# PieSil/CUDA-spectral-ray-tracer

Measured on AMD Instinct MI355X. Metric: Mray/s, higher is better.
Workload: dtype f32; 1 GPU; random-spheres tri scene (4802 tris, 9603 BVH nodes), 1920x1080, 1024 spp, depth 16; scene_id=100, tiles=8x8 px per wave, rank = tile % n_gpus, gather=none (1 GPU), launch_mode=one process, one GPU

## Files before the change

cuda-spectral-ray-tracer_amd/binding.py:

```python
import ctypes as C
import os

_HERE = os.path.dirname(os.path.abspath(__file__))
LIB_PATH = os.environ.get("SRT_LIB_PATH") or os.path.join(_HERE, "libsrt_hip.so")

N_CIE = 95
TILE_PLANES = 9
TILE_LANES = 64

SCENE_CORNELL, SCENE_PRISM, SCENE_TRIS, SCENE_RANDOM_SPHERES, SCENE_MESH100K = 0, 1, 2, 100, 101
BVH_REFERENCE, BVH_SAH = 0, 1
MAT_LAMBERTIAN, MAT_METALLIC, MAT_DIELECTRIC, MAT_EMISSIVE, MAT_NO_MAT = 0, 1, 2, 4, 6


class TriIn(C.Structure):
    _fields_ = [("v0", C.c_float * 3), ("v1", C.c_float * 3), ("v2", C.c_float * 3),
                ("mat_index", C.c_uint32), ("aa_plane", C.c_uint32)]


class Material(C.Structure):
    _fields_ = [("col", C.c_float * 3), ("reflection_fuzz", C.c_float), ("material_type", C.c_uint32),
                ("spectral_distribution", C.c_float * N_CIE), ("emission_power", C.c_float),
                ("sellmeier_B", C.c_float * 3), ("sellmeier_C", C.c_float * 3)]

# ... 118 lines not shown
    "srt_denoise_estimate_last_ms": (_i, [_vp, _fp]),
    "srt_denoise_features_mv": (_i, [_vp, C.POINTER(DenoiseVG), _fp, _fp, _fp, _fp, _u32, _u32]),
    "srt_denoise_mv_kat": (_i, [_vp, C.POINTER(DenoiseVG), _fp, _fp, C.POINTER(_u32), _fp, _u32, _u32, _fp, _fp]),
    "srt_accum_reset_streams": (_i, [_vp, _u32]),
    "srt_accum_streams": (_i, [_vp, C.POINTER(_u32)]),
    "srt_set_gather_planes": (_i, [_vp, _u32]),
    "srt_tile_buffer": (_i, [_vp, C.POINTER(_vp), C.POINTER(_sz), C.POINTER(_u32), C.POINTER(_u32)]),
    "srt_copy_tile_buffer": (_i, [_vp, _vp, _vp]),
    "srt_scatter_tiles": (_i, [_vp, _vp, _vp]),
    "srt_dev_fb": (_i, [_vp, C.POINTER(_vp), C.POINTER(_vp), C.POINTER(_vp), C.POINTER(_sz)]),
    "srt_read_fb": (_i, [_vp, _fp, _fp, _fp]),
    "srt_read_fb_rowmajor": (_i, [_vp, _fp, _fp, _fp, _u32, _u32]),
    "srt_read_fb_aux": (_i, [_vp, _i, _fp, _fp, _fp]),
    "srt_get_tile_costs": (_i, [_vp, C.POINTER(C.c_uint32), _sz]),
    "srt_order_children_by_profile": (_i, [_vp, _vp, C.c_uint32, C.c_uint32, C.c_uint32, C.c_uint32, C.c_uint32, C.POINTER(C.c_uint32)]),
    "srt_pixels_per_lane": (_i, [_vp, _u32, _u32, _u32, C.POINTER(C.c_double)]),
    "srt_tune_tree_for_throughput": (_i, [_vp, _vp, _u32, _u32, _u32, _u32, _i, C.POINTER(TreeTuning)]),
    "srt_get_stats": (_i, [_vp, C.POINTER(Stats)]),
    "srt_set_count_traversal": (_i, [_vp, _i]),
    "srt_get_wave_debug": (_i, [_vp, C.POINTER(C.c_uint32), _sz]),
    "srt_last_kernel_ms": (_i, [_vp, C.POINTER(_f)]),
    "srt_trace_rays": (_i, [_vp, _fp, _sz, _fp]),
    "srt_device_op_sweep": (_i, [_vp, _i, _fp, _fp, _sz, _fp]),
    "srt_order_tiles_kat": (_i, [_vp, C.POINTER(_u32), _u32, _u32, _u32, _u32, C.POINTER(_u32), _sz, C.POINTER(_u32), C.POINTER(_u32)]),
    "srt_read_tile_schedule": (_i, [_vp, _i, C.POINTER(_u32), _sz, C.POINTER(TileScheduleInfo)]),
    "srt_calibrate": (_i, [_vp, _i, _u32, _u32, C.POINTER(Calibration)]),
    "srt_ctx_device": (_i, [_vp]),
    "srt_ctx_cu_count": (_i, [_vp]),
    "srt_comm_init_all": (_i, [C.POINTER(_i), _i, C.POINTER(_vp)]),
    "srt_comm_unique_id": (_i, [C.POINTER(C.c_ubyte)]),
    "srt_comm_init_rank": (_i, [_vp, C.POINTER(C.c_ubyte), _u32, _u32, C.POINTER(_vp)]),
    "srt_comm_available": (_i, []),
    "srt_comm_set_gather_planes": (_i, [_vp, _u32]),
    "srt_comm_last_gather_ms": (_i, [_vp, C.POINTER(_f)]),
    "srt_comm_destroy": (None, [_vp]),
    "srt_comm_last_error": (C.c_char_p, [_vp]),
    "srt_comm_world": (_u32, [_vp]),
    "srt_comm_local_count": (_u32, [_vp]),
    "srt_comm_ctx": (_vp, [_vp, _u32]),
    "srt_comm_root_ctx": (_vp, [_vp]),
    "srt_comm_upload_scene": (_i, [_vp, _vp]),
    "srt_comm_set_camera": (_i, [_vp, C.POINTER(CameraData)]),
    "srt_comm_init_device_params": (_i, [_vp, _u32, _u32, _u32, _u32, _u32, _u32, _u32, _u32, _u64]),
    "srt_render_frame_multi": (_i, [_vp, _u32, _u32, _u32, _u32]),
    "srt_comm_accum_reset": (_i, [_vp]),
    "srt_render_frame_multi_accum": (_i, [_vp, _u32, _u32, _u32, _u32, _u32]),
# ... 56 lines not shown
```

cuda-spectral-ray-tracer_amd/csrc/srt_capi.cpp:

```cpp
#include <dlfcn.h>
#include <hip/hip_runtime.h>
#include <stdint.h>
#include <stdlib.h>
#include <string.h>

#include <algorithm>
#include <cmath>
#include <cstddef>
#include <string>
#include <vector>

#include "srt_host.h"
#include "srt_internal.h"

using namespace srt;

#ifndef SRT_FRINGE_STRIDE_L2
#define SRT_FRINGE_STRIDE_L2 96
#endif
static constexpr uint32_t kFringeStrideL2 = SRT_FRINGE_STRIDE_L2;
static constexpr uint32_t kScoreShadeL2 = 320u, kScoreFringeL2 = 800u;

struct DeviceBuffer {
    void *ptr = nullptr;
// ... 1679 lines not shown
    RenderParams p;
    fill_params(c, p);
    HIP_TRY_AS(c, "srt_trace_rays", launch_trace(p, d_in.as<float>(), n, d_out.as<float>(), nullptr));
    HIP_TRY_AS(c, "srt_trace_rays", hipDeviceSynchronize());
    HIP_TRY_AS(c, "srt_trace_rays", hipMemcpy(out, d_out.ptr, 4 * n * sizeof(float), hipMemcpyDeviceToHost));
    return SRT_OK;
}

int srt_device_op_sweep(srt_ctx *c, int which, const float *a, const float *b, size_t n, float *out) {
    if (!c || !a || !b || !out) return fail(c, SRT_ERR_INVALID, "srt_device_op_sweep: null argument");
    if (n == 0) return SRT_OK;
    HIP_TRY(c, hipSetDevice(c->device));
    DeviceBuffer buf;
    HIP_TRY_AS(c, "srt_device_op_sweep", buf.reserve(3 * n * sizeof(float)));
    float *d = buf.as<float>();
    HIP_TRY_AS(c, "srt_device_op_sweep", hipMemcpy(d, a, n * sizeof(float), hipMemcpyHostToDevice));
    HIP_TRY_AS(c, "srt_device_op_sweep", hipMemcpy(d + n, b, n * sizeof(float), hipMemcpyHostToDevice));
    HIP_TRY_AS(c, "srt_device_op_sweep", launch_op_sweep(which, d, d + n, n, d + 2 * n, nullptr));
    HIP_TRY_AS(c, "srt_device_op_sweep", hipDeviceSynchronize());
    HIP_TRY_AS(c, "srt_device_op_sweep", hipMemcpy(out, d + 2 * n, n * sizeof(float), hipMemcpyDeviceToHost));
    return SRT_OK;
}

int srt_order_tiles_kat(srt_ctx *c, const uint32_t *cost, uint32_t n, uint32_t n_waves, uint32_t split_load_pct, uint32_t order_max_pct,
                        uint32_t *rows_out, size_t rows_cap, uint32_t *sorted_out, uint32_t *info_out) {
    if (!c || !cost || !rows_out || !sorted_out || !info_out) return fail(c, SRT_ERR_INVALID, "srt_order_tiles_kat: null argument");
    if (n == 0 || n > (1u << 20)) return fail(c, SRT_ERR_INVALID, "srt_order_tiles_kat: n must be in 1 .. 2^20");
    if (rows_cap < (size_t)n * 64 + 64) return fail(c, SRT_ERR_INVALID, "srt_order_tiles_kat: rows_cap must be at least 64 * n + 64 (the largest queue and 64 guard words)");
    HIP_TRY(c, hipSetDevice(c->device));
    DeviceBuffer d_cost, d_rows, d_sorted, d_info;
    HIP_TRY_AS(c, "srt_order_tiles_kat", d_cost.reserve(TileSchedule::cost_bytes(n)));
    HIP_TRY_AS(c, "srt_order_tiles_kat", d_rows.reserve(rows_cap * sizeof(uint32_t)));
    HIP_TRY_AS(c, "srt_order_tiles_kat", d_sorted.reserve(n * sizeof(uint32_t)));
    HIP_TRY_AS(c, "srt_order_tiles_kat", d_info.reserve(4 * sizeof(uint32_t)));
    HIP_TRY_AS(c, "srt_order_tiles_kat", hipMemcpy(d_cost.ptr, cost, TileSchedule::cost_bytes(n), hipMemcpyHostToDevice));
    HIP_TRY_AS(c, "srt_order_tiles_kat", hipMemset(d_rows.ptr, 0xff, rows_cap * sizeof(uint32_t)));
    HIP_TRY_AS(c, "srt_order_tiles_kat", hipMemset(d_sorted.ptr, 0xff, n * sizeof(uint32_t)));
    HIP_TRY_AS(c, "srt_order_tiles_kat", hipMemset(d_info.ptr, 0xff, 4 * sizeof(uint32_t)));
    HIP_TRY_AS(c, "srt_order_tiles_kat", launch_order_tiles(d_cost.as<uint32_t>(), d_sorted.as<uint32_t>(), d_rows.as<uint32_t>(), n, n_waves, split_load_pct,
                                                            d_info.as<uint32_t>(), order_max_pct, nullptr));
    HIP_TRY_AS(c, "srt_order_tiles_kat", hipDeviceSynchronize());
    HIP_TRY_AS(c, "srt_order_tiles_kat", hipMemcpy(rows_out, d_rows.ptr, rows_cap * sizeof(uint32_t), hipMemcpyDeviceToHost));
    HIP_TRY_AS(c, "srt_order_tiles_kat", hipMemcpy(sorted_out, d_sorted.ptr, n * sizeof(uint32_t), hipMemcpyDeviceToHost));
    HIP_TRY_AS(c, "srt_order_tiles_kat", hipMemcpy(info_out, d_info.ptr, 4 * sizeof(uint32_t), hipMemcpyDeviceToHost));
    return SRT_OK;
}
// ... 56 lines not shown
```

cuda-spectral-ray-tracer_amd/csrc/srt_device.h:

```cpp
#pragma once
#include <hip/hip_runtime.h>
#include <stdint.h>

#include "srt_color_consts.h"
#include "srt_powf.h"

namespace srt {

constexpr int kCieSamples = 95;
constexpr int kWavelengths = 7;
constexpr float kLambdaMin = 360.0f;
constexpr float kLambdaMax = 830.0f;
constexpr float kEpsilon = 0.0001f;
constexpr float kFltMax = 3.402823466e+38f;

__device__ __noinline__ static float dev_powf(float x, float y) { return srt_powf(x, y); }

struct V3 { float x, y, z; };
__device__ __forceinline__ V3 mk(float x, float y, float z) { V3 r; r.x = x; r.y = y; r.z = z; return r; }
__device__ __forceinline__ V3 operator+(V3 a, V3 b) { return mk(a.x + b.x, a.y + b.y, a.z + b.z); }
__device__ __forceinline__ V3 operator-(V3 a, V3 b) { return mk(a.x - b.x, a.y - b.y, a.z - b.z); }
__device__ __forceinline__ V3 operator-(V3 a) { return mk(-a.x, -a.y, -a.z); }
__device__ __forceinline__ V3 operator*(float t, V3 v) { return mk(t * v.x, t * v.y, t * v.z); }
__device__ __forceinline__ float dot(V3 a, V3 b) { return a.x * b.x + a.y * b.y + a.z * b.z; }
__device__ __forceinline__ float length_squared(V3 v) { return v.x * v.x + v.y * v.y + v.z * v.z; }
__device__ __forceinline__ V3 unit_vector(V3 v) { float k = 1.0f / sqrtf(length_squared(v)); return k * v; }
__device__ __forceinline__ V3 reflect(V3 v, V3 n) { return v - (2.0f * dot(v, n)) * n; }
__device__ __forceinline__ V3 refract(V3 uv, V3 n, float etai_over_etat) {
    float cos_theta = fminf(dot(-uv, n), 1.0f);
    V3 r_out_perp = etai_over_etat * (uv + cos_theta * n);
    V3 r_out_parallel = (-sqrtf(fabsf(1.0f - length_squared(r_out_perp)))) * n;
    return r_out_perp + r_out_parallel;
}

__device__ __forceinline__ float inside_min2(float a1, float a2, uint32_t sign) {
    return __builtin_elementwise_minimum(__uint_as_float(__float_as_uint(a1) ^ sign), __uint_as_float(__float_as_uint(a2) ^ sign));
}
__device__ __forceinline__ bool inside_min3(float m12, float a3, uint32_t sign) {
    return __builtin_elementwise_minimum(m12, __uint_as_float(__float_as_uint(a3) ^ sign)) >= 0.f;
}

__device__ __forceinline__ bool near_zero(V3 v) {
    const float s = 1e-8f;
    return (fabsf(v.x) < s) && (fabsf(v.y) < s) && (fabsf(v.z) < s);
}

struct Rng { uint32_t d, v0, v1, v2, v3, v4; };
#ifndef SRT_XOR3
#define SRT_XOR3 1
#endif
#ifndef SRT_ASM_RNG
#define SRT_ASM_RNG 1
#endif

// ... 94 lines not shown
        : "s80", "s81", "vcc");
}
__device__ __forceinline__ V3 random_in_unit_sphere(Rng &s) {
#if SRT_ASM_RNG
    {
        float x, y, z, len2;
        rng_sphere_loop_asm(s, x, y, z, len2);
        return mk(x, y, z);
    }
#endif
    for (;;) {
        float x = rng_pm1(s);
        float y = rng_pm1(s);
        float z = rng_pm1(s);
        V3 p = mk(x, y, z);
        if (length_squared(p) < 1.0f) return p;
    }
}

__device__ __forceinline__ V3 random_unit_vector(Rng &s) {
#if SRT_ASM_RNG
    float x, y, z, len2;
    rng_sphere_loop_asm(s, x, y, z, len2);
    const float k = 1.0f / sqrtf(len2);
    return k * mk(x, y, z);
#else
    return unit_vector(random_in_unit_sphere(s));
#endif
}

__device__ __forceinline__ void interp_coords(float lambda, int &offset, float &weight) {
    lambda -= kLambdaMin;
    lambda *= ((float)kCieSamples - 1) / (kLambdaMax - kLambdaMin);
    offset = (int)lambda;
    if (offset < 0) offset = 0;
    if (offset > kCieSamples - 2) offset = kCieSamples - 2;
    weight = lambda - (float)offset;
}
__device__ __forceinline__ float interp_pair(float2 pr, float weight) { return (1.0f - weight) * pr.x + weight * pr.y; }

__device__ __forceinline__ float hero_draw(Rng &s) { return rng_range(s, kLambdaMin, kLambdaMax); }
__device__ __forceinline__ void hero_expand(float hero, float (&wl)[kWavelengths]) {
    const float step = (kLambdaMax - kLambdaMin) / (float)kWavelengths;
    wl[0] = hero;
    float lambda = hero;
#pragma unroll
    for (int i = 1; i < kWavelengths; i++) {
// ... 7 lines not shown
}

__device__ __forceinline__ float correct_channel(float value) {
    return value < 0.0f ? 0.0f
         : (value < 0.0031308f ? 12.92f * value
         : (value < 1.0f ? ((1.055f * dev_powf(value, 0.416666f)) - 0.055f) : 1.0f));
}
struct SrgbPixel { V3 lin, q; };
__device__ __forceinline__ SrgbPixel xyz_mean_to_srgb(V3 c) {
    const float r_lin = (SRT_XYZ2RGB_00 * c.x) + (SRT_XYZ2RGB_01 * c.y) + (SRT_XYZ2RGB_02 * c.z);
    const float g_lin = (SRT_XYZ2RGB_10 * c.x) + (SRT_XYZ2RGB_11 * c.y) + (SRT_XYZ2RGB_12 * c.z);
    const float b_lin = (SRT_XYZ2RGB_20 * c.x) + (SRT_XYZ2RGB_21 * c.y) + (SRT_XYZ2RGB_22 * c.z);
    const float r = correct_channel(r_lin), g = correct_channel(g_lin), b = correct_channel(b_lin);
    SrgbPixel o;
    o.lin = mk(r, g, b);
    o.q = mk((float)(int)(r * 255.99f), (float)(int)(g * 255.99f), (float)(int)(b * 255.99f));
    return o;
}

__device__ __forceinline__ float sellmeier_index(float b0, float b1, float b2, float c0, float c1, float c2, float lambda) {
    lambda *= 1e-3f;
    float l2 = lambda * lambda;
    float index = 1.0f + (b0 * l2) / (l2 - c0) + (b1 * l2) / (l2 - c1) + (b2 * l2) / (l2 - c2);
    return sqrtf(index);
}
__device__ __forceinline__ float reflectance(float cosine, float ref_idx) {
    float r0 = (1.0f - ref_idx) / (1.0f + ref_idx);
    r0 = r0 * r0;
    return r0 + (1.0f - r0) * srt_pow5f(1.0f - cosine);
}

constexpr uint32_t kTriWIsY = 1u, kTriHIsZ = 2u, kTriClockwise = 4u;

__device__ __forceinline__ bool tri_test(const float4 *__restrict__ tris, int tri, V3 o, V3 d, float tmin, float tmax,
                                         float &t_out) {
    const float4 a = tris[3 * tri + 0];
    const V3 n = mk(a.x, a.y, a.z);
    float denom = dot(n, d);
    if (fabsf(denom) < 1e-8f) return false;
    float t = (a.w - dot(n, o)) / denom;
    if (!(tmin <= t && t <= tmax)) return false;
    const float4 b = tris[3 * tri + 1];
    const float4 c = tris[3 * tri + 2];
    const uint32_t flags = __float_as_uint(c.z);
    const bool wy = flags & kTriWIsY, hz = flags & kTriHIsZ;
    float pw = (wy ? o.y : o.x) + t * (wy ? d.y : d.x);
    float ph = (hz ? o.z : o.y) + t * (hz ? d.z : d.y);
// ... 554 lines not shown
```

cuda-spectral-ray-tracer_amd/csrc/srt_internal.h:

```cpp
#pragma once
#include <hip/hip_runtime.h>
#include <stdint.h>
#include <stddef.h>

struct srt_ctx;
extern "C" int srt_internal_init_device_params(srt_ctx *c, uint32_t tx, uint32_t ty, uint32_t bx, uint32_t by, uint32_t chunk_w, uint32_t chunk_h,
                                               uint32_t spp, uint32_t bounce_limit, uint64_t seed, int wait);

extern "C" uint32_t srt_internal_gather_planes(const srt_ctx *c);

namespace srt {

constexpr int kTilePlanes = 9;
constexpr int kTileGroups = 3;
constexpr int kGroupPlanes = 3;
constexpr int kTileLanes = 64;
constexpr int kCounters = 32;

constexpr uint32_t kQueueTileBits = 22, kQueueTileMask = (1u << kQueueTileBits) - 1u;
constexpr uint32_t kQueuePartShift = kQueueTileBits, kQueuePartMask = 63u;
constexpr uint32_t kQueueLevelShift = 28, kQueueLevelMask = 7u;

struct RenderParams {
    const float4 *nodes;
// ... 174 lines not shown
};
hipError_t launch_denoise_level_dev(const DenoiseLevelDevParams &p, hipStream_t st);
hipError_t launch_denoise_dev_out(const float4 *payload, float *out_dev, uint32_t channels, uint32_t groups, size_t n, hipStream_t st);
constexpr uint32_t kMaxDevelopChannels = 16;
struct DevelopParams {
    const float *film, *response;
    float *out;
    float scale;
    uint32_t channels;
    uint32_t n_lanes, tx, ty, bx;
    uint32_t w, h;
};
uint32_t develop_padded_channels(uint32_t channels);
hipError_t launch_develop(const DevelopParams &p, hipStream_t st);
hipError_t launch_develop_srgb(const float *xyz, float *out_lin, float *out_q, uint32_t samples, size_t n, hipStream_t st);
hipError_t launch_order_tiles(const uint32_t *cost, uint32_t *sorted, uint32_t *rows, uint32_t n, uint32_t n_waves,
                              uint32_t split_load_pct, uint32_t *queue_info, uint32_t order_max_pct, hipStream_t st);
hipError_t launch_scatter(const ScatterParams &p, hipStream_t st);
hipError_t launch_unswizzle(const float *const src[3], float *const dst[3], uint32_t tx, uint32_t ty, uint32_t bx, uint32_t by,
                            uint32_t n_cols, uint32_t n_rows, uint32_t offx, uint32_t offy, uint32_t image_width,
                            uint32_t image_height, hipStream_t st);
hipError_t launch_trace(const RenderParams &p, const float *rays, size_t n, float *out, hipStream_t st);
hipError_t launch_op_sweep(int which, const float *a, const float *b, size_t n, float *out, hipStream_t st);
hipError_t launch_calib(int kind, uint32_t n_blocks, uint32_t threads, uint32_t iters, float *sink, unsigned long long *cycles, const float4 *table,
                        uint32_t n_records, hipStream_t st);
int calib_kinds();
bool render_narrow_refs(int n_records, const PlanKnobs &k);
bool render_paired_variant(bool tree_is_paired, bool narrow, bool all_cached);
size_t render_lds_bytes(int stack_depth, int waves_per_block, int n_cached, int n_records, const PlanKnobs &k);
void render_launch_shape(int stack_depth, int n_records, int n_inner, const PlanKnobs &k, int &waves_per_block, int &n_cached);
struct LaunchPlan { int waves_per_block, blocks_per_cu, waves_per_cu, waves_per_eu, n_cached; bool all_cached; };
void render_launch_plan(int stack_depth, int n_records, int n_inner, const PlanKnobs &k, LaunchPlan &lp);
struct RenderGrid { int waves_per_block; uint32_t n_blocks, waves; };
RenderGrid render_launch_grid(const LaunchPlan &lp, uint32_t n_cu, uint32_t waves_per_cu_override, uint32_t queue_rows_bound);

}
```

cuda-spectral-ray-tracer_amd/csrc/srt_kernels.hip:

```cpp
#include <algorithm>
#include <stdlib.h>

#include "srt_color_consts.h"
#include "srt_kernel_common.h"

namespace srt {

#ifndef SRT_INNER_BURST
#define SRT_INNER_BURST 8
#endif
#ifndef SRT_BURST_DROP
#define SRT_BURST_DROP 3
#endif
#ifndef SRT_ASM_BURST
#define SRT_ASM_BURST 2
#endif
#ifndef SRT_INNER_BURST_L2
#define SRT_INNER_BURST_L2 4
#endif
#ifndef SRT_ASM_BURST_L2
#define SRT_ASM_BURST_L2 1
#endif
#ifndef SRT_BURST_DROP_L2
#define SRT_BURST_DROP_L2 2
// ... 66 lines not shown
    Rng s;
    rng_seed(s, seed + idx);
    rng[0 * (size_t)n_lanes + idx] = s.d;
    rng[1 * (size_t)n_lanes + idx] = s.v0;
    rng[2 * (size_t)n_lanes + idx] = s.v1;
    rng[3 * (size_t)n_lanes + idx] = s.v2;
    rng[4 * (size_t)n_lanes + idx] = s.v3;
    rng[5 * (size_t)n_lanes + idx] = s.v4;
}

__device__ __forceinline__ bool adaptive_converged(float s1, float s2, uint32_t n_samples, uint32_t min_spp, float rel_tol, float abs_tol) {
    const float n = (float)n_samples;
    const float mean = s1 / n;
    const float mm = mean * mean;
    float v = s2 / n - mm;
    v = v > 0.0f ? v : 0.0f;
    const float var_mean = v / (n - 1.0f);
    const float tol = rel_tol * mean + abs_tol;
    const float tt = tol * tol;
    const bool finite = __builtin_isfinite(s1) && __builtin_isfinite(s2) && __builtin_isfinite(mm) && __builtin_isfinite(tt);
    return n_samples >= min_spp && finite && var_mean <= tt;
}

template <int MODE, bool NARROW, bool ALL_CACHED, bool PAIRED>
__global__ __launch_bounds__(1024) void render_kernel(const RenderParams P) {
    constexpr bool COUNT = (MODE == 1);
    constexpr bool PROBE = (MODE == 2);
    constexpr bool ITERS = COUNT || PROBE;
    constexpr bool ACCUM = (MODE == 3 || MODE == 4 || MODE == 5 || MODE == 7 || MODE == 8 || MODE == 9);
    constexpr bool ADAPT = (MODE == 4 || MODE == 8);
    constexpr bool FILM = (MODE == 5 || MODE == 9);
    constexpr bool STREAMS = (MODE == 6);
    constexpr bool FEATURES = (MODE == 7 || MODE == 8 || MODE == 9);
    constexpr bool S2_MEM = ADAPT && !NARROW && !ALL_CACHED && !PAIRED;
    extern __shared__ float4 lds4[];
    lds_uniforms *U = (lds_uniforms *)lds4;
    float4 *s_cmf = lds4 + kLdsUniF4;
    constexpr bool narrow = NARROW;
    const uint32_t nc = (uint32_t)P.n_cached;
    float4 *s_q0 = lds4 + kLdsTablesF4, *s_q1 = s_q0 + nc, *s_q2 = s_q1 + nc;
    uint32_t *s_r0 = reinterpret_cast<uint32_t *>(s_q2 + nc), *s_r1 = s_r0 + nc;
    const size_t cache_b = (((size_t)nc * (narrow ? 52u : 56u)) + 15u) & ~(size_t)15u;
    char *s_stack_base = reinterpret_cast<char *>(lds4 + kLdsTablesF4) + cache_b;
    const uint32_t lane = threadIdx.x & 63u;
    const uint32_t wave = threadIdx.x >> 6;

// ... 130 lines not shown
                            const float m = fminf(fminf(fmaxf(x0, x1), fmaxf(y0, y1)), fmaxf(z0, z1));
                            if (e <= m && e > tv.c) atomicAdd(&prof.cnt[up], 1u);
                            k = up >> 1;
                        }
                    }
                    const uint32_t srec = __umul24((uint32_t)tv.hit, 48u);
                    const f4v s0 = buf_load16(shade_rsrc, srec), s1 = buf_load16(shade_rsrc, srec + 16u), s2 = buf_load16(shade_rsrc, srec + 32u);
                    const V3 n_geo = mk(s0.x, s0.y, s0.z);
                    const V3 hp = ro + tv.c * rd;
                    const bool front_face = dot(rd, n_geo) < 0;
                    const V3 n = front_face ? n_geo : -n_geo;
                    const uint32_t mat = __float_as_uint(s0.w);
                    const uint32_t mtype = __float_as_uint(s1.x);
                    const float fuzz = s1.y;

                    V3 scatter_direction = mk(0.f, 0.f, 0.f);
                    float eps_sign = 1.0f;
                    bool did_scatter = true;
                    const V3 unit_in = unit_vector(rd);
                    if (mtype == 4u) {
                        did_scatter = false;
                    } else if (mtype == 2u) {
                        float ir = sellmeier_index(s1.z, s1.w, s2.x, s2.y, s2.z, s2.w, wl[0]);
                        float refraction_ratio = front_face ? (1.0f / ir) : ir;
                        float cos_theta = fminf(dot(-unit_in, n), 1.0f);
                        float sin_theta = sqrtf(1.0f - cos_theta * cos_theta);
                        bool cannot_refract = refraction_ratio * sin_theta > 1.0f;
                        if (!cannot_refract)
                            cannot_refract = reflectance(cos_theta, refraction_ratio) > rng_uniform(rs);
                        if (cannot_refract) {
                            scatter_direction = reflect(unit_in, n);
                        } else {
                            scatter_direction = refract(unit_in, n, refraction_ratio);
                            eps_sign = -1.0f;
                            valid = 1;
                        }
                    } else {
                        const V3 ruv = random_unit_vector(rs);
                        if (mtype == 1u) {
                            V3 reflected = reflect(unit_in, n);
                            scatter_direction = reflected + fuzz * ruv;
                            did_scatter = dot(scatter_direction, n) > 0;
                            if (!did_scatter) valid = 0;
                        } else {
                            scatter_direction = n + ruv;
                            if (near_zero(scatter_direction)) scatter_direction = n;
                        }
                    }
                    if constexpr (FEATURES) {
// ... 261 lines not shown
                if (!(U->defocus_angle <= 0.0f)) {
                    float dx, dy;
#if SRT_ASM_RNG
                    rng_disk_loop_asm(rs, dx, dy);
#else
                    for (;;) {
                        dx = rng_pm1(rs);
                        dy = rng_pm1(rs);
                        if ((dx * dx + dy * dy) + 0.0f * 0.0f < 1.0f) break;
                    }
#endif
                    origin = (cam_center + dx * mk(U->disk_u[0], U->disk_u[1], U->disk_u[2])) +
                             dy * mk(U->disk_v[0], U->disk_v[1], U->disk_v[2]);
                }
                ro = origin;
                rd = pixel_sample - origin;
                hero = hero_draw(rs);
#pragma unroll
                for (int k = 0; k < kWavelengths; k++) pw[k] = 1.0f;
                valid = kWavelengths;
                sample++;
                bounce = 0;
                have_path = true;
                if (P.bounce_limit > 0) begin_trav = true;
                else { valid = 0;
                       have_path = false;  }
            }

            if (begin_trav) {
                n_rays++;
                inv = mk(1.0f / rd.x, 1.0f / rd.y, 1.0f / rd.z);
                ray_near_addresses(ns, inv, tv.nf);
                (void)trav_begin<ITERS>(tv, stack_base<NARROW>(my_stack), P.tris, P.root_ref, ro, rd, ts);
            }
        }

        if (COUNT) { const unsigned long long now = __builtin_amdgcn_s_memtime(); t_shade += now - t_mark; t_mark = now; }
        if (__ballot(!dead) == 0ull) break;
        const unsigned long long alive_mask = __ballot(!dead && !parked);
        if (alive_mask == 0ull) continue;
        const uint32_t n_alive = (uint32_t)__popcll(alive_mask);
        const uint32_t n_inner_u = (uint32_t)P.n_inner;
        if (!COUNT && n_alive == 1u) {
            while (__ballot(tv.node >= 0) != 0ull) {
                if (tv.node >= 0) {
                    if ((uint32_t)tv.node < n_inner_u) trav_step_inner<ITERS, NARROW, ALL_CACHED>(tv, ns, ro, inv, my_stack, ts);
                    else trav_step_fringe<ITERS, NARROW, PAIRED>(tv, ns, ro, rd, inv, my_stack, ts);
                }
            }
            continue;
        }
        if (!ITERS && NARROW && ALL_CACHED && kInnerBurst == 8 && kBurstDrop == 3u && SRT_ASM_BURST == 2) {
            while (inner_phase_asm(tv, ns, ro, inv, n_inner_u, n_alive, w_shade, w_fringe) != 0u) {
                if (tv.node >= (int)n_inner_u) trav_step_fringe<ITERS, NARROW, PAIRED>(tv, ns, ro, rd, inv, my_stack, ts);
            }
        } else
// ... 277 lines not shown
    case 17: r = srt_pow5f(x); break;
    case 18: r = rng_unit_from_bits(__float_as_uint(x)); break;
    case 19: r = rng_pm1_from_bits(__float_as_uint(x)); break;
    case 20: { float m = inside_min2(x, y, 0u); asm volatile("" : "+v"(m)); r = inside_min3(m, z, 0u) ? 1.f : 0.f; } break;
    case 21: { float m = inside_min2(x, y, 0x80000000u); asm volatile("" : "+v"(m)); r = inside_min3(m, z, 0x80000000u) ? 1.f : 0.f; } break;
    case 22: r = n >= 6u ? sellmeier_index(b[0], b[1], b[2], b[3], b[4], b[5], x) : 0.f; break;
    case 23: case 24: case 25: case 26: case 27: {
        Rng s; rng_seed(s, (uint64_t)__float_as_uint(x));
        float px, py, pz, l2; rng_sphere_loop_asm(s, px, py, pz, l2);
        r = which == 23 ? px : which == 24 ? py : which == 25 ? pz : which == 26 ? l2 : __uint_as_float(s.d ^ (s.v0 * 3u) ^ (s.v1 * 5u) ^ (s.v2 * 7u) ^ (s.v3 * 11u) ^ (s.v4 * 13u));
    } break;
    case 28: case 29: case 30: {
        Rng s; rng_seed(s, (uint64_t)__float_as_uint(x));
        float px, py; rng_disk_loop_asm(s, px, py);
        r = which == 28 ? px : which == 29 ? py : __uint_as_float(s.d ^ (s.v0 * 3u) ^ (s.v1 * 5u) ^ (s.v2 * 7u) ^ (s.v3 * 11u) ^ (s.v4 * 13u));
    } break;
    case 31: case 32: case 33: {
        Rng s; rng_seed(s, (uint64_t)__float_as_uint(x));
        const uint32_t steps = __float_as_uint(y);
        uint32_t xo = 0u, sm = 0u;
        for (uint32_t i = 0; i < steps; i++) { const uint32_t v = rng_next(s); xo ^= v; sm += v * (2u * i + 1u); }
        r = __uint_as_float(which == 31 ? xo : which == 32 ? sm : s.d ^ (s.v0 * 3u) ^ (s.v1 * 5u) ^ (s.v2 * 7u) ^ (s.v3 * 11u) ^ (s.v4 * 13u));
    } break;
    default: r = 0.f;
    }
    out[k] = r;
}

hipError_t launch_init_rng(uint32_t *rng, uint32_t n_lanes, uint64_t seed, hipStream_t st) {
    if (n_lanes == 0) return hipSuccess;
    hipLaunchKernelGGL(init_rng_kernel, dim3((n_lanes + 255) / 256), dim3(256), 0, st, rng, n_lanes, seed);
    return hipGetLastError();
}

template <int MODE, bool NARROW, bool ALL_CACHED, bool PAIRED = false>
static hipError_t launch_render_cached(const RenderParams &p_in, const LaunchPlan &lp, const PlanKnobs &knobs, uint32_t n_cu, hipStream_t st) {
    RenderParams p = p_in;
    const RenderGrid grid = render_launch_grid(lp, n_cu, p.waves_per_cu_override, p.queue_rows_bound);
    p.n_cached = lp.n_cached;
    const size_t lds = render_lds_bytes(p.stack_depth, grid.waves_per_block, lp.n_cached, p.n_records, knobs);
    {
        const hipError_t ae = hipFuncSetAttribute(reinterpret_cast<const void *>(&render_kernel<MODE, NARROW, ALL_CACHED, PAIRED>), hipFuncAttributeMaxDynamicSharedMemorySize, (int)kLdsBudget);
        if (ae != hipSuccess) return ae;
    }
    hipLaunchKernelGGL((render_kernel<MODE, NARROW, ALL_CACHED, PAIRED>), dim3(grid.n_blocks), dim3(64 * grid.waves_per_block), lds, st, p);
    return hipGetLastError();
}

template <int MODE, bool NARROW>
// ... 29 lines not shown
    return hipGetLastError();
}

hipError_t launch_scatter(const ScatterParams &p, hipStream_t st) {
    if (p.n_tiles == 0) return hipSuccess;
    hipLaunchKernelGGL(scatter_tiles_kernel, dim3(p.n_tiles), dim3(64), 0, st, p);
    return hipGetLastError();
}

hipError_t launch_unswizzle(const float *const src[3], float *const dst[3], uint32_t tx, uint32_t ty, uint32_t bx, uint32_t by,
                            uint32_t n_cols, uint32_t n_rows, uint32_t offx, uint32_t offy, uint32_t image_width,
                            uint32_t image_height, hipStream_t st) {
    const uint32_t n = tx * ty * bx * by;
    if (n == 0) return hipSuccess;
    hipLaunchKernelGGL(unswizzle_kernel, dim3((n + 255) / 256), dim3(256), 0, st, src[0], src[1], src[2], dst[0], dst[1], dst[2],
                       tx, ty, bx, by, n_cols, n_rows, offx, offy, image_width, image_height);
    return hipGetLastError();
}

hipError_t launch_trace(const RenderParams &p, const float *rays, size_t n, float *out, hipStream_t st) {
    if (n == 0) return hipSuccess;
    const size_t lds = stack_slots(p.stack_depth) * 64 * 4;
    hipLaunchKernelGGL(trace_rays_kernel, dim3((uint32_t)((n + 63) / 64)), dim3(64), lds, st, p, rays, (uint32_t)n, out);
    return hipGetLastError();
}

hipError_t launch_op_sweep(int which, const float *a, const float *b, size_t n, float *out, hipStream_t st) {
    if (n == 0) return hipSuccess;
    hipLaunchKernelGGL(op_sweep_kernel, dim3((uint32_t)((n + 255) / 256)), dim3(256), 0, st, which, a, b, (uint32_t)n, out);
    return hipGetLastError();
}

template <int>
__global__ void accum_header_kernel(AccumHeader *dst, float *sums, uint32_t spp_total) {
    if (threadIdx.x == 0) { dst->sums = sums; dst->spp_total = spp_total; dst->pad = 0u; }
}

hipError_t launch_accum_header(AccumHeader *dst, float *sums, uint32_t spp_total, hipStream_t st) {
    hipLaunchKernelGGL(accum_header_kernel<0>, dim3(1), dim3(64), 0, st, dst, sums, spp_total);
    return hipGetLastError();
}

template <int>
__global__ __launch_bounds__(256) void adapt_flag_kernel(const AdaptQueueParams P) {
    const uint32_t lane = threadIdx.x & 63u;
    const uint32_t wave = (blockIdx.x * blockDim.x + threadIdx.x) >> 6, n_waves = (gridDim.x * blockDim.x) >> 6;
// ... 127 lines not shown
```

cuda-spectral-ray-tracer_amd/renderer.py:

```python
import contextlib
import ctypes as C

import numpy as np

from . import binding as B

DEFAULT_TX, DEFAULT_TY = 28, 16
FEATURE_CHANNELS = 8
FILM_SAMPLES = 95


def reference_grid(chunk_w, chunk_h, tx=DEFAULT_TX, ty=DEFAULT_TY):
    return chunk_w // tx + 1, chunk_h // ty + 1


class Renderer:
    def __init__(self, device=0, _borrowed=None):
        if _borrowed is not None:
            self._h, self._owned = C.c_void_p(_borrowed), False
            self.device = B.lib().srt_ctx_device(self._h)
        else:
            h = C.c_void_p()
            B.check(B.lib().srt_create(int(device), C.byref(h)))
            self._h, self._owned = h, True
# ... 324 lines not shown
        cal = B.Calibration()
        self._ck(B.lib().srt_calibrate(self._h, kind, waves_per_simd, iters, C.byref(cal)))
        n_simd = cal.n_cu * 4
        total = cal.instr_per_wave * cal.n_waves
        clock_ghz = cal.wave_cycles_max / (cal.wall_ms * 1e-3) / 1e9
        return dict(kind=kind, waves_per_simd=cal.waves_per_simd, n_cu=cal.n_cu, wave_cycles_min=cal.wave_cycles_min,
                    wave_cycles_mean=cal.wave_cycles_mean, wave_cycles_max=cal.wave_cycles_max, wall_ms=cal.wall_ms,
                    instr_per_wave=cal.instr_per_wave,
                    instr_per_cycle_per_simd=cal.instr_per_wave * cal.waves_per_simd / cal.wave_cycles_max,
                    instr_per_cycle_per_simd_mean_wave=cal.instr_per_wave * cal.waves_per_simd / cal.wave_cycles_mean,
                    instr_per_s=total / (cal.wall_ms * 1e-3), clock_ghz=clock_ghz, n_simd=n_simd)

    def trace_rays(self, rays):
        rays = np.ascontiguousarray(rays, np.float32).reshape(-1, 6)
        out = np.zeros((rays.shape[0], 4), np.float32)
        self._ck(B.lib().srt_trace_rays(self._h, B.fptr(rays), rays.shape[0], B.fptr(out)))
        return out

    def op_sweep(self, which, a, b):
        a = np.ascontiguousarray(a, np.float32); b = np.ascontiguousarray(b, np.float32)
        out = np.zeros_like(a)
        self._ck(B.lib().srt_device_op_sweep(self._h, which, B.fptr(a), B.fptr(b), a.size, B.fptr(out)))
        return out

    def order_tiles_kat(self, cost, n_waves, split_load_pct=200, order_max_pct=0, guard=64):
        cost = np.ascontiguousarray(cost, np.uint32)
        n = cost.size // 2
        u32p = C.POINTER(C.c_uint32)
        rows, order, info = np.zeros(64 * n + guard, np.uint32), np.zeros(n, np.uint32), np.zeros(4, np.uint32)
        self._ck(B.lib().srt_order_tiles_kat(self._h, cost.ctypes.data_as(u32p), n, int(n_waves), int(split_load_pct), int(order_max_pct),
                                             rows.ctypes.data_as(u32p), rows.size, order.ctypes.data_as(u32p), info.ctypes.data_as(u32p)))
        return rows, order, info

    def tile_schedule(self, which=0):
        _, _, tl, _ = self.tile_buffer()
        rows, info = np.zeros(64 * tl, np.uint32), B.TileScheduleInfo()
        self._ck(B.lib().srt_read_tile_schedule(self._h, int(which), rows.ctypes.data_as(C.POINTER(C.c_uint32)), rows.size, C.byref(info)))
        return rows[:info.n_rows].copy(), {name: getattr(info, name) for name, _ in B.TileScheduleInfo._fields_ if name != "reserved"}


class Comm:

    def __init__(self, handle, renderers, owns):
        self._h, self.renderers, self._owns = handle, renderers, owns
        self.world = B.lib().srt_comm_world(handle)

# ... 565 lines not shown
```

include/srt_c_api.h:

```cpp
#ifndef SRT_C_API_H
#define SRT_C_API_H

#include <stddef.h>
#include <stdint.h>

#ifdef __cplusplus
extern "C" {
#endif

#define SRT_API __attribute__((visibility("default")))

#define SRT_N_CIE_SAMPLES 95
#define SRT_N_RAY_WAVELENGTHS 7
#define SRT_DEFAULT_SEED 1984u
#define SRT_DEFAULT_TX 28u
#define SRT_DEFAULT_TY 16u

typedef enum {
    SRT_OK = 0,
    SRT_ERR_INVALID = -1,
    SRT_ERR_NO_DEVICE = -2,
    SRT_ERR_HIP = -3,
    SRT_ERR_BVH = -4,
    SRT_ERR_UNSUPPORTED = -5,
// ... 162 lines not shown
SRT_API int srt_read_fb_rowmajor(srt_ctx *ctx, float *r, float *g, float *b, uint32_t image_width, uint32_t image_height);
SRT_API int srt_read_fb_aux(srt_ctx *ctx, int which, float *p0, float *p1, float *p2);

SRT_API int srt_get_tile_costs(srt_ctx *ctx, uint32_t *out, size_t n);
SRT_API int srt_order_children_by_profile(srt_ctx *ctx, srt_scene *scene, uint32_t width, uint32_t height, uint32_t spp,
                                          uint32_t bounce_limit, uint32_t min_samples, uint32_t *n_swapped);
SRT_API int srt_pixels_per_lane(const srt_ctx *ctx, uint32_t width, uint32_t height, uint32_t world, double *out);
typedef struct srt_tree_tuning {
    double   pixels_per_lane;
    uint32_t throughput_bound;
    uint32_t reinsertion;
    uint32_t probe_width, probe_height, probe_spp;
    uint32_t nodes_swapped;
    int32_t  order_status;
} srt_tree_tuning;
SRT_API int srt_tune_tree_for_throughput(srt_ctx *ctx, srt_scene *scene, uint32_t width, uint32_t height, uint32_t world,
                                         uint32_t bounce_limit, int only_if_throughput_bound, srt_tree_tuning *out);
SRT_API int srt_get_stats(srt_ctx *ctx, srt_stats *out);
SRT_API int srt_set_count_traversal(srt_ctx *ctx, int on);
SRT_API int srt_get_wave_debug(srt_ctx *ctx, uint32_t *out, size_t n_waves);
SRT_API int srt_last_kernel_ms(srt_ctx *ctx, float *ms);
SRT_API int srt_trace_rays(srt_ctx *ctx, const float *rays, size_t n, float *out);
SRT_API int srt_device_op_sweep(srt_ctx *ctx, int which, const float *a, const float *b, size_t n, float *out);
SRT_API int srt_order_tiles_kat(srt_ctx *ctx, const uint32_t *cost, uint32_t n, uint32_t n_waves, uint32_t split_load_pct,
                                uint32_t order_max_pct, uint32_t *rows_out, size_t rows_cap, uint32_t *sorted_out, uint32_t *info_out);
typedef struct srt_tile_schedule_info {
    uint32_t tiles_local;
    uint32_t n_rows;
    uint32_t cost_max;
    uint32_t n_waves_plan;
    uint32_t split_load_pct;
    uint32_t order_max_pct;
    uint32_t streams;
    uint32_t reserved;
} srt_tile_schedule_info;
SRT_API int srt_read_tile_schedule(srt_ctx *ctx, int which, uint32_t *rows_out, size_t rows_cap, srt_tile_schedule_info *info);

SRT_API int srt_ctx_device(const srt_ctx *ctx);
SRT_API int srt_ctx_cu_count(const srt_ctx *ctx);

#define SRT_COMM_ID_BYTES 128
typedef struct srt_comm srt_comm;
SRT_API int srt_comm_init_all(const int *devices, int n, srt_comm **out);
SRT_API int srt_comm_unique_id(unsigned char id[SRT_COMM_ID_BYTES]);
SRT_API int srt_comm_init_rank(srt_ctx *ctx, const unsigned char id[SRT_COMM_ID_BYTES], uint32_t rank, uint32_t world, srt_comm **out);
SRT_API int srt_comm_available(void);
// ... 40 lines not shown
```

Measured before the change: 16090 Mray/s.

## Replace IEEE div/sqrt with short bit-exact chains plus wave-uniform fallback

Replaces 1/x and sqrtf in the hot traversal and shading paths with short hardware rcp/sqrt sequences. Each uses one Newton step or neighbour-candidate correction and falls back to the full IEEE path only when some lane in the wave has an out-of-range exponent. It also forces a few uniform params (bounce_limit, root_ref) into scalar registers. An exhaustive device sweep kernel and API are added to confirm bit-exactness. The aim is to cut the long compiler-generated scaled division/sqrt sequences, at the cost of an extra ballot per call.

```diff
diff --git a/cuda-spectral-ray-tracer_amd/binding.py b/cuda-spectral-ray-tracer_amd/binding.py
--- a/cuda-spectral-ray-tracer_amd/binding.py
+++ b/cuda-spectral-ray-tracer_amd/binding.py
@@ -164,6 +164,7 @@
     "srt_last_kernel_ms": (_i, [_vp, C.POINTER(_f)]),
     "srt_trace_rays": (_i, [_vp, _fp, _sz, _fp]),
     "srt_device_op_sweep": (_i, [_vp, _i, _fp, _fp, _sz, _fp]),
+    "srt_device_exact_sweep": (_i, [_vp, _i, _i, _u32, _u64, C.POINTER(_u64), C.POINTER(_u32)]),
     "srt_order_tiles_kat": (_i, [_vp, C.POINTER(_u32), _u32, _u32, _u32, _u32, C.POINTER(_u32), _sz, C.POINTER(_u32), C.POINTER(_u32)]),
     "srt_read_tile_schedule": (_i, [_vp, _i, C.POINTER(_u32), _sz, C.POINTER(TileScheduleInfo)]),
     "srt_calibrate": (_i, [_vp, _i, _u32, _u32, C.POINTER(Calibration)]),
diff --git a/cuda-spectral-ray-tracer_amd/csrc/srt_capi.cpp b/cuda-spectral-ray-tracer_amd/csrc/srt_capi.cpp
--- a/cuda-spectral-ray-tracer_amd/csrc/srt_capi.cpp
+++ b/cuda-spectral-ray-tracer_amd/csrc/srt_capi.cpp
@@ -1725,6 +1725,25 @@
     return SRT_OK;
 }
 
+int srt_device_exact_sweep(srt_ctx *c, int which, int order, uint32_t first, uint64_t count, uint64_t *n_bad, uint32_t *first_bad) {
+    if (!c || !n_bad || !first_bad) return fail(c, SRT_ERR_INVALID, "srt_device_exact_sweep: null argument");
+    if (which < 0 || which > 1 || order < 0 || order > 1) return fail(c, SRT_ERR_INVALID, "srt_device_exact_sweep: which and order must be 0 or 1");
+    if (count > (1ull << 32)) return fail(c, SRT_ERR_INVALID, "srt_device_exact_sweep: count must be at most 2^32");
+    *n_bad = 0; *first_bad = 0xffffffffu;
+    if (count == 0) return SRT_OK;
+    HIP_TRY(c, hipSetDevice(c->device));
+    DeviceBuffer buf;
+    HIP_TRY_AS(c, "srt_device_exact_sweep", buf.reserve(4 * sizeof(uint32_t)));
+    uint32_t h[4] = {0u, 0u, 0xffffffffu, 0u};
+    HIP_TRY_AS(c, "srt_device_exact_sweep", hipMemcpy(buf.ptr, h, sizeof h, hipMemcpyHostToDevice));
+    HIP_TRY_AS(c, "srt_device_exact_sweep", launch_exact_sweep(which, order, first, count, buf.as<uint32_t>(), nullptr));
+    HIP_TRY_AS(c, "srt_device_exact_sweep", hipDeviceSynchronize());
+    HIP_TRY_AS(c, "srt_device_exact_sweep", hipMemcpy(h, buf.ptr, sizeof h, hipMemcpyDeviceToHost));
+    *n_bad = (uint64_t)h[0] | ((uint64_t)h[1] << 32);
+    *first_bad = h[2];
+    return SRT_OK;
+}
+
 int srt_order_tiles_kat(srt_ctx *c, const uint32_t *cost, uint32_t n, uint32_t n_waves, uint32_t split_load_pct, uint32_t order_max_pct,
                         uint32_t *rows_out, size_t rows_cap, uint32_t *sorted_out, uint32_t *info_out) {
     if (!c || !cost || !rows_out || !sorted_out || !info_out) return fail(c, SRT_ERR_INVALID, "srt_order_tiles_kat: null argument");
diff --git a/cuda-spectral-ray-tracer_amd/csrc/srt_device.h b/cuda-spectral-ray-tracer_amd/csrc/srt_device.h
--- a/cuda-spectral-ray-tracer_amd/csrc/srt_device.h
+++ b/cuda-spectral-ray-tracer_amd/csrc/srt_device.h
@@ -15,6 +15,58 @@
 constexpr float kFltMax = 3.402823466e+38f;
 
 __device__ __noinline__ static float dev_powf(float x, float y) { return srt_powf(x, y); }
+
+#ifndef SRT_SHORT_RCP
+#define SRT_SHORT_RCP 1
+#endif
+#ifndef SRT_SHORT_SQRT
+#define SRT_SHORT_SQRT 1
+#endif
+__device__ __forceinline__ float rcp_chain(float x) {
+    float r = __builtin_amdgcn_rcpf(x);
+    const float e = __builtin_fmaf(-x, r, 1.0f);
+    r = __builtin_fmaf(e, r, r);
+    return __builtin_amdgcn_div_fixupf(r, x, 1.0f);
+}
+__device__ __forceinline__ int rcp_exponent(float x) { return __builtin_amdgcn_frexp_expf(x); }
+__device__ __forceinline__ bool rcp_outside(int e) { return (uint32_t)(e + 125) > 251u; }
+__device__ __forceinline__ bool wave_any(bool outside) { return __builtin_expect(__builtin_amdgcn_ballot_w64(outside) != 0ull, 0); }
+__device__ __forceinline__ float rcp_rn(float x) {
+#if SRT_SHORT_RCP
+    float r = rcp_chain(x);
+    if (wave_any(rcp_outside(rcp_exponent(x)))) r = 1.0f / x;
+    return r;
+#else
+    return 1.0f / x;
+#endif
+}
+__device__ __forceinline__ float sqrt_chain(float x) {
+    const float s = __builtin_amdgcn_sqrtf(x);
+    const float lo = __uint_as_float(__float_as_uint(s) - 1u), hi = __uint_as_float(__float_as_uint(s) + 1u);
+    const float r_lo = __builtin_fmaf(-lo, s, x), r_hi = __builtin_fmaf(-hi, s, x);
+    float o = r_lo <= 0.0f ? lo : s;
+    o = r_hi > 0.0f ? hi : o;
+    return o;
+}
+__device__ __forceinline__ bool sqrt_outside(float x) { return fabsf(x) < 0x1p-96f; }
+__device__ __forceinline__ float sqrt_rn(float x) {
+#if SRT_SHORT_SQRT
+    float r = sqrt_chain(x);
+    if (wave_any(sqrt_outside(x))) r = sqrtf(x);
+    return r;
+#else
+    return sqrtf(x);
+#endif
+}
+__device__ __forceinline__ float rcp_sqrt_rn(float x) {
+#if SRT_SHORT_RCP && SRT_SHORT_SQRT
+    float r = rcp_chain(sqrt_chain(x));
+    if (wave_any(sqrt_outside(x))) r = 1.0f / sqrtf(x);
+    return r;
+#else
+    return rcp_rn(sqrt_rn(x));
+#endif
+}
 
 struct V3 { float x, y, z; };
 __device__ __forceinline__ V3 mk(float x, float y, float z) { V3 r; r.x = x; r.y = y; r.z = z; return r; }
@@ -24,12 +76,23 @@
 __device__ __forceinline__ V3 operator*(float t, V3 v) { return mk(t * v.x, t * v.y, t * v.z); }
 __device__ __forceinline__ float dot(V3 a, V3 b) { return a.x * b.x + a.y * b.y + a.z * b.z; }
 __device__ __forceinline__ float length_squared(V3 v) { return v.x * v.x + v.y * v.y + v.z * v.z; }
-__device__ __forceinline__ V3 unit_vector(V3 v) { float k = 1.0f / sqrtf(length_squared(v)); return k * v; }
+__device__ __forceinline__ V3 unit_vector(V3 v) { float k = rcp_sqrt_rn(length_squared(v)); return k * v; }
+__device__ __forceinline__ V3 rcp3_rn(V3 v) {
+#if SRT_SHORT_RCP
+    const int ex = rcp_exponent(v.x), ey = rcp_exponent(v.y), ez = rcp_exponent(v.z);
+    const bool outside = rcp_outside(max(max(ex, ey), ez)) || rcp_outside(min(min(ex, ey), ez));
+    V3 r = mk(rcp_chain(v.x), rcp_chain(v.y), rcp_chain(v.z));
+    if (wave_any(outside)) r = mk(1.0f / v.x, 1.0f / v.y, 1.0f / v.z);
+    return r;
+#else
+    return mk(1.0f / v.x, 1.0f / v.y, 1.0f / v.z);
+#endif
+}
 __device__ __forceinline__ V3 reflect(V3 v, V3 n) { return v - (2.0f * dot(v, n)) * n; }
 __device__ __forceinline__ V3 refract(V3 uv, V3 n, float etai_over_etat) {
     float cos_theta = fminf(dot(-uv, n), 1.0f);
     V3 r_out_perp = etai_over_etat * (uv + cos_theta * n);
-    V3 r_out_parallel = (-sqrtf(fabsf(1.0f - length_squared(r_out_perp)))) * n;
+    V3 r_out_parallel = (-sqrt_rn(fabsf(1.0f - length_squared(r_out_perp)))) * n;
     return r_out_perp + r_out_parallel;
 }
 
@@ -170,7 +233,7 @@
 #if SRT_ASM_RNG
     float x, y, z, len2;
     rng_sphere_loop_asm(s, x, y, z, len2);
-    const float k = 1.0f / sqrtf(len2);
+    const float k = rcp_sqrt_rn(len2);
     return k * mk(x, y, z);
 #else
     return unit_vector(random_in_unit_sphere(s));
@@ -224,7 +287,7 @@
     lambda *= 1e-3f;
     float l2 = lambda * lambda;
     float index = 1.0f + (b0 * l2) / (l2 - c0) + (b1 * l2) / (l2 - c1) + (b2 * l2) / (l2 - c2);
-    return sqrtf(index);
+    return sqrt_rn(index);
 }
 __device__ __forceinline__ float reflectance(float cosine, float ref_idx) {
     float r0 = (1.0f - ref_idx) / (1.0f + ref_idx);
diff --git a/cuda-spectral-ray-tracer_amd/csrc/srt_internal.h b/cuda-spectral-ray-tracer_amd/csrc/srt_internal.h
--- a/cuda-spectral-ray-tracer_amd/csrc/srt_internal.h
+++ b/cuda-spectral-ray-tracer_amd/csrc/srt_internal.h
@@ -220,6 +220,7 @@
                             uint32_t image_height, hipStream_t st);
 hipError_t launch_trace(const RenderParams &p, const float *rays, size_t n, float *out, hipStream_t st);
 hipError_t launch_op_sweep(int which, const float *a, const float *b, size_t n, float *out, hipStream_t st);
+hipError_t launch_exact_sweep(int which, int order, uint32_t first, uint64_t count, uint32_t *res, hipStream_t st);
 hipError_t launch_calib(int kind, uint32_t n_blocks, uint32_t threads, uint32_t iters, float *sink, unsigned long long *cycles, const float4 *table,
                         uint32_t n_records, hipStream_t st);
 int calib_kinds();
diff --git a/cuda-spectral-ray-tracer_amd/csrc/srt_kernels.hip b/cuda-spectral-ray-tracer_amd/csrc/srt_kernels.hip
--- a/cuda-spectral-ray-tracer_amd/csrc/srt_kernels.hip
+++ b/cuda-spectral-ray-tracer_amd/csrc/srt_kernels.hip
@@ -112,6 +112,16 @@
     return n_samples >= min_spp && finite && var_mean <= tt;
 }
 
+#ifndef SRT_RARE_SCALARS
+#define SRT_RARE_SCALARS 1
+#endif
+__device__ __forceinline__ uint32_t rare_scalar(uint32_t v) {
+#if SRT_RARE_SCALARS
+    asm volatile("" : "+s"(v));
+#endif
+    return v;
+}
+
 template <int MODE, bool NARROW, bool ALL_CACHED, bool PAIRED>
 __global__ __launch_bounds__(1024) void render_kernel(const RenderParams P) {
     constexpr bool COUNT = (MODE == 1);
@@ -288,9 +298,9 @@
                         did_scatter = false;
                     } else if (mtype == 2u) {
                         float ir = sellmeier_index(s1.z, s1.w, s2.x, s2.y, s2.z, s2.w, wl[0]);
-                        float refraction_ratio = front_face ? (1.0f / ir) : ir;
+                        float refraction_ratio = front_face ? rcp_rn(ir) : ir;
                         float cos_theta = fminf(dot(-unit_in, n), 1.0f);
-                        float sin_theta = sqrtf(1.0f - cos_theta * cos_theta);
+                        float sin_theta = sqrt_rn(1.0f - cos_theta * cos_theta);
                         bool cannot_refract = refraction_ratio * sin_theta > 1.0f;
                         if (!cannot_refract)
                             cannot_refract = reflectance(cos_theta, refraction_ratio) > rng_uniform(rs);
@@ -598,16 +608,16 @@
                 sample++;
                 bounce = 0;
                 have_path = true;
-                if (P.bounce_limit > 0) begin_trav = true;
+                if (rare_scalar(P.bounce_limit) > 0) begin_trav = true;
                 else { valid = 0;
                        have_path = false;  }
             }
 
             if (begin_trav) {
                 n_rays++;
-                inv = mk(1.0f / rd.x, 1.0f / rd.y, 1.0f / rd.z);
+                inv = rcp3_rn(rd);
                 ray_near_addresses(ns, inv, tv.nf);
-                (void)trav_begin<ITERS>(tv, stack_base<NARROW>(my_stack), P.tris, P.root_ref, ro, rd, ts);
+                (void)trav_begin<ITERS>(tv, stack_base<NARROW>(my_stack), P.tris, (int)rare_scalar((uint32_t)P.root_ref), ro, rd, ts);
             }
         }
 
@@ -931,9 +941,28 @@
         for (uint32_t i = 0; i < steps; i++) { const uint32_t v = rng_next(s); xo ^= v; sm += v * (2u * i + 1u); }
         r = __uint_as_float(which == 31 ? xo : which == 32 ? sm : s.d ^ (s.v0 * 3u) ^ (s.v1 * 5u) ^ (s.v2 * 7u) ^ (s.v3 * 11u) ^ (s.v4 * 13u));
     } break;
+    case 34: r = rcp_rn(x); break;
+    case 35: r = sqrt_rn(x); break;
     default: r = 0.f;
     }
     out[k] = r;
+}
+
+__global__ void exact_sweep_kernel(int which, int order, uint32_t first, unsigned long long count, uint32_t *res) {
+    const unsigned long long stride = (unsigned long long)gridDim.x * blockDim.x;
+    const unsigned long long trips = (count + stride - 1ull) / stride;
+    unsigned long long k = (unsigned long long)blockIdx.x * blockDim.x + threadIdx.x;
+    for (unsigned long long t = 0; t < trips; t++, k += stride) {
+        const uint32_t idx = first + (uint32_t)(k < count ? k : count - 1ull);
+        const uint32_t bits = order ? __builtin_bitreverse32(idx) : idx;
+        const float x = __uint_as_float(bits);
+        const float want = which ? sqrtf(x) : 1.0f / x;
+        const float got = which ? sqrt_rn(x) : rcp_rn(x);
+        if (__float_as_uint(want) != __float_as_uint(got) && k < count) {
+            atomicAdd((unsigned long long *)res, 1ull);
+            atomicMin(res + 2, bits);
+        }
+    }
 }
 
 hipError_t launch_init_rng(uint32_t *rng, uint32_t n_lanes, uint64_t seed, hipStream_t st) {
@@ -1009,6 +1038,13 @@
     if (n == 0) return hipSuccess;
     const size_t lds = stack_slots(p.stack_depth) * 64 * 4;
     hipLaunchKernelGGL(trace_rays_kernel, dim3((uint32_t)((n + 63) / 64)), dim3(64), lds, st, p, rays, (uint32_t)n, out);
+    return hipGetLastError();
+}
+
+hipError_t launch_exact_sweep(int which, int order, uint32_t first, uint64_t count, uint32_t *res, hipStream_t st) {
+    if (count == 0) return hipSuccess;
+    const uint64_t blocks = (count + 255u) / 256u;
+    hipLaunchKernelGGL(exact_sweep_kernel, dim3((uint32_t)(blocks < 8192u ? blocks : 8192u)), dim3(256), 0, st, which, order, first, (unsigned long long)count, res);
     return hipGetLastError();
 }
 
diff --git a/cuda-spectral-ray-tracer_amd/renderer.py b/cuda-spectral-ray-tracer_amd/renderer.py
--- a/cuda-spectral-ray-tracer_amd/renderer.py
+++ b/cuda-spectral-ray-tracer_amd/renderer.py
@@ -370,6 +370,11 @@
         out = np.zeros_like(a)
         self._ck(B.lib().srt_device_op_sweep(self._h, which, B.fptr(a), B.fptr(b), a.size, B.fptr(out)))
         return out
+
+    def exact_sweep(self, which, order, first=0, count=1 << 32):
+        n_bad, first_bad = C.c_uint64(0), C.c_uint32(0)
+        self._ck(B.lib().srt_device_exact_sweep(self._h, which, order, first, count, C.byref(n_bad), C.byref(first_bad)))
+        return n_bad.value, first_bad.value
 
     def order_tiles_kat(self, cost, n_waves, split_load_pct=200, order_max_pct=0, guard=64):
         cost = np.ascontiguousarray(cost, np.uint32)
diff --git a/include/srt_c_api.h b/include/srt_c_api.h
--- a/include/srt_c_api.h
+++ b/include/srt_c_api.h
@@ -208,6 +208,7 @@
 SRT_API int srt_last_kernel_ms(srt_ctx *ctx, float *ms);
 SRT_API int srt_trace_rays(srt_ctx *ctx, const float *rays, size_t n, float *out);
 SRT_API int srt_device_op_sweep(srt_ctx *ctx, int which, const float *a, const float *b, size_t n, float *out);
+SRT_API int srt_device_exact_sweep(srt_ctx *ctx, int which, int order, uint32_t first, uint64_t count, uint64_t *n_bad, uint32_t *first_bad);
 SRT_API int srt_order_tiles_kat(srt_ctx *ctx, const uint32_t *cost, uint32_t n, uint32_t n_waves, uint32_t split_load_pct,
                                 uint32_t order_max_pct, uint32_t *rows_out, size_t rows_cap, uint32_t *sorted_out, uint32_t *info_out);
 typedef struct srt_tile_schedule_info {
diff --git a/profiles/shading_trims2/experiments/chain_sweep.hip b/profiles/shading_trims2/experiments/chain_sweep.hip
--- /dev/null
+++ b/profiles/shading_trims2/experiments/chain_sweep.hip
@@ -0,0 +1,107 @@
+#include <hip/hip_runtime.h>
+#include <cstdio>
+#include <cstdint>
+#include <cstdlib>
+
+__device__ __forceinline__ float fixup1(float q, float x) { return __builtin_amdgcn_div_fixupf(q, x, 1.0f); }
+
+template <int V> __device__ __forceinline__ float rcp_short(float x) {
+    float r = __builtin_amdgcn_rcpf(x);
+    if (V == 0) return fixup1(r, x);
+    float e = __builtin_fmaf(-x, r, 1.0f);
+    r = __builtin_fmaf(e, r, r);
+    if (V == 1) return fixup1(r, x);
+    if (V == 2) {
+        e = __builtin_fmaf(-x, r, 1.0f);
+        return fixup1(__builtin_fmaf(e, r, r), x);
+    }
+    if (V == 3) {
+        float q = r;
+        e = __builtin_fmaf(-x, q, 1.0f);
+        q = __builtin_fmaf(e, r, q);
+        e = __builtin_fmaf(-x, q, 1.0f);
+        return fixup1(__builtin_fmaf(e, r, q), x);
+    }
+    if (V == 4) {
+        e = __builtin_fmaf(-x, r, 1.0f);
+        return __builtin_fmaf(e, r, r);
+    }
+    return r;
+}
+
+template <int V> __device__ __forceinline__ float sqrt_short(float x) {
+    if (V == 0 || V == 1) {
+        float s = __builtin_amdgcn_sqrtf(x);
+        float sm = __uint_as_float(__float_as_uint(s) - 1u), sp = __uint_as_float(__float_as_uint(s) + 1u);
+        float rm = __builtin_fmaf(-sm, s, x), rp = __builtin_fmaf(-sp, s, x);
+        float o = (rm <= 0.0f) ? sm : s;
+        o = (rp > 0.0f) ? sp : o;
+        if (V == 1) o = __builtin_amdgcn_class(x, 0x260) ? x : o;
+        return o;
+    }
+    if (V == 2) {
+        float s = __builtin_amdgcn_sqrtf(x);
+        float h = 0.5f * __builtin_amdgcn_rsqf(x);
+        float r = __builtin_fmaf(-s, s, x);
+        return __builtin_fmaf(r, h, s);
+    }
+    if (V == 3) {
+        float y = __builtin_amdgcn_rsqf(x);
+        float g = x * y, h = 0.5f * y;
+        float r = __builtin_fmaf(-g, g, x);
+        return __builtin_fmaf(r, h, g);
+    }
+    return x;
+}
+
+template <int FN, int V> __global__ void sweep(uint32_t *hist, uint32_t *first_bad) {
+    const uint64_t n = 1ull << 32;
+    for (uint64_t i = (uint64_t)blockIdx.x * blockDim.x + threadIdx.x; i < n; i += (uint64_t)gridDim.x * blockDim.x) {
+        const uint32_t b = (uint32_t)i;
+        const float x = __uint_as_float(b);
+        float want, got;
+        if (FN == 0) { want = 1.0f / x; got = rcp_short<V>(x); }
+        else { want = sqrtf(x); got = sqrt_short<V>(x); }
+        if (__float_as_uint(want) != __float_as_uint(got)) {
+            atomicAdd(&hist[b >> 23], 1u);
+            atomicMin(first_bad, b);
+        }
+    }
+}
+
+template <int FN, int V> static void run(const char *name) {
+    uint32_t *d_hist, *d_first;
+    hipMalloc(&d_hist, 512 * 4); hipMalloc(&d_first, 4);
+    hipMemset(d_hist, 0, 512 * 4); hipMemset(d_first, 0xff, 4);
+    sweep<FN, V><<<4096, 256>>>(d_hist, d_first);
+    uint32_t hist[512], first;
+    if (hipMemcpy(hist, d_hist, sizeof hist, hipMemcpyDeviceToHost) != hipSuccess) { printf("%s: HIP error\n", name); exit(1); }
+    hipMemcpy(&first, d_first, 4, hipMemcpyDeviceToHost);
+    uint64_t total = 0;
+    for (int i = 0; i < 512; i++) total += hist[i];
+    printf("%s: total mismatches %llu first 0x%08x\n", name, (unsigned long long)total, first);
+    int start = -1;
+    for (int i = 0; i <= 512; i++) {
+        const bool bad = i < 512 && hist[i];
+        if (bad && start < 0) start = i;
+        if (!bad && start >= 0) {
+            uint64_t s = 0; for (int k = start; k < i; k++) s += hist[k];
+            printf("    buckets 0x%03x..0x%03x (sign %d exp %d..%d): %llu\n", start, i - 1, start >> 8, start & 255, (i - 1) & 255, (unsigned long long)s);
+            start = -1;
+        }
+    }
+    hipFree(d_hist); hipFree(d_first);
+}
+
+int main() {
+    run<0, 0>("rcp V0 rcp+fixup");
+    run<0, 1>("rcp V1 one step+fixup");
+    run<0, 2>("rcp V2 two steps+fixup");
+    run<0, 3>("rcp V3 compiler chain unscaled");
+    run<0, 4>("rcp V4 two steps no fixup");
+    run<1, 0>("sqrt V0 candidates, no class");
+    run<1, 1>("sqrt V1 candidates + class");
+    run<1, 2>("sqrt V2 sqrt+rsq newton");
+    run<1, 3>("sqrt V3 rsq g/h");
+    return 0;
+}
```

After: 16200 Mray/s (median of 6 runs). About the same (+0.7%).
